# graphdeco-inria/editable-gaussian-reflections

Measured on AMD Instinct MI355X. Metric: Mrays/s fwd+bwd @1080p, 1M Gaussians, higher is better.
Workload: dtype f32; 1 GPU; BASELINE config C: synthetic dense-init room+spheres cloud, HEADLINE variant = init (literal dense-init opacity 0.1 (config.py:44): Kc ~ 22 per ray, bounces mostly die), N=1000000, 1920x1080, one training iteration: export + update_bvh + forward + backward + grad import, num_bounces=2, jitter on, reference default config; variant=init, gaussians=1000000, width=1920, height=1080, parallelism=image tiles x1 + 1 all-reduce of the launch's [22N] gradients, team_help=product default (on)

## Files before the change

editable-gaussian-reflections_amd/csrc/backward_task.inc:

```
        const uint32_t task = v.bwd_order[tq];
        uint32_t blk = v.task_last_block[(size_t)step * (BATCH ? v.num_tasks * v.batch_frames : v.num_tasks) + task];
        if (blk == 0xFFFFFFFFu) continue;
        uint32_t tb = task, bframe = 0u;
        if constexpr (BATCH) tb = batch_base_task(v, task), bframe = v.batch_frame0 + (task >> v.task_shift) % v.batch_frames;
        (void)bframe;
        const TaskGeom tg = task_geom(v, tb, lane);
        const StateRef S = state_of(v, task, lane);
        uint32_t steps_done = tg.inside ? f2u(S.ld(F_STEPS)) : 0u;
        uint32_t nhits = (tg.inside && (uint32_t)step < steps_done && blk != 0xFFFFFFFFu) ? f2u(S.ld(SF(step, S_NHITS))) : 0u;
        const uint32_t max_hits = wave_max_u32(nhits);
        if (max_hits == 0) continue;
#if defined(EGR_TASK_TIMES) && EGR_TASK_TIMES == 8
        if (PRIMARY) bw_rows0 = max_hits;
#endif

        f3 dL_rgb = mk3(0, 0, 0), dL_n = mk3(0, 0, 0), dL_f0 = mk3(0, 0, 0);
        float dL_depth = 0.0f, dL_rough = 0.0f;
        f3 ro = mk3(0, 0, 0), rd = mk3(0, 0, 1);
        f3 rem_rgb = mk3(0, 0, 0), rem_n = mk3(0, 0, 0), rem_f0 = mk3(0, 0, 0);
        float rem_depth = 0.0f, rem_rough = 0.0f, T_minus_Ttot = 0.0f;
        if (nhits > 0) {
            const uint32_t pid = tg.pixel_id;
            const float third = 1.0f / 3.0f;
            if (PRIMARY && BATCH) {
// ... 18 lines not shown
                dL_rgb = mk3(third * sign1(o_rgb.x - td[0]), third * sign1(o_rgb.y - td[1]), third * sign1(o_rgb.z - td[2])) * *v.cfg.loss_weight_diffuse;
                dL_depth = sign1(o_depth - v.fb.target_depth[pid]) * *v.cfg.loss_weight_depth;
                dL_n = mk3(third * sign1(o_n.x - tn[0]), third * sign1(o_n.y - tn[1]), third * sign1(o_n.z - tn[2])) * *v.cfg.loss_weight_normal;
                dL_f0 = mk3(third * sign1(o_f0.x - tf[0]), third * sign1(o_f0.y - tf[1]), third * sign1(o_f0.z - tf[2])) * *v.cfg.loss_weight_f0;
                dL_rough = sign1(o_rough - v.fb.target_roughness[pid]) * *v.cfg.loss_weight_roughness;
                uint32_t seed = tea4(pid, (uint32_t)*v.meta.total_num_calls);
                ro = mk3(v.cam.origin[0], v.cam.origin[1], v.cam.origin[2]);
                rd = primary_direction(v, tg.px, tg.py, *v.cfg.jitter_primary_rays != 0, seed, view_size, v.cam.rotation_w2c);
            } else {
                f3 spec = mk3(0, 0, 0);
                for (int j = 1; j < num_bounces + 1; j++)
                    if ((uint32_t)j < steps_done) spec = spec + S.ld3(SF(j, S_RGB));
                f3 t_spec;
                if constexpr (BATCH) {
                    const float *p = v.batch_targets[1];
                    const size_t P = v.num_pixels, q = (size_t)bframe * 3 * P + pid;
                    t_spec = p ? mk3(p[q], p[q + P], p[q + 2 * P]) : mk3(0, 0, 0);
                } else {
                    const float *ts = v.fb.target_specular + 3 * (size_t)pid;
                    t_spec = mk3(ts[0], ts[1], ts[2]);
                }
                float down = powf(1.0f - S.ld(SF(step - 1, S_ROUGH)), EGR_ROUGHNESS_DOWNWEIGHT_GRAD_POWER);
                dL_rgb = (mk3(third * sign1(spec.x - t_spec.x), third * sign1(spec.y - t_spec.y), third * sign1(spec.z - t_spec.z)) *
                          *v.cfg.loss_weight_specular) * down;
                dL_rgb = dL_rgb * S.ld3(SF(step - 1, S_THR));
                ro = S.ld3(SF(step - 1, S_NEXT_O));
                rd = S.ld3(SF(step - 1, S_NEXT_D));
            }
            rem_rgb = S.ld3(SF(step, S_REM_RGB)), rem_n = S.ld3(SF(step, S_REM_NORMAL)), rem_f0 = S.ld3(SF(step, S_REM_F0));
            rem_depth = S.ld(SF(step, S_REM_DEPTH)), rem_rough = S.ld(SF(step, S_REM_ROUGH));
            T_minus_Ttot = S.ld(SF(step, S_T)) - S.ld(SF(step, S_TTOT));
        }

        auto hit_geometry = [&](uint32_t pos, const float4 &a2, const f3 &ro, const f3 &rd, float dL_dalpha, auto &gx) { hit_geometry_fn(v, exp_power, eps_scale_grad, pos, a2, ro, rd, dL_dalpha, gx); };

        if constexpr (!PRIMARY) {
            table_dirty = true;
            bdl[lane] = dL_rgb.x, bdl[EGR_WAVE + lane] = dL_rgb.y, bdl[2 * EGR_WAVE + lane] = dL_rgb.z;
            bray[lane] = ro.x, bray[EGR_WAVE + lane] = ro.y, bray[2 * EGR_WAVE + lane] = ro.z, bray[3 * EGR_WAVE + lane] = rd.x, bray[4 * EGR_WAVE + lane] = rd.y, bray[5 * EGR_WAVE + lane] = rd.z;
            f3 prev_rgb = mk3(0, 0, 0), w_rgb = mk3(0, 0, 0);
            const uint32_t nblocks = (max_hits + EGR_HIT_BLOCK_ROWS - 1) / EGR_HIT_BLOCK_ROWS;
            EGR_BWD_SYNC();
            for (uint32_t b = nblocks; b-- > 0;) {
                const float4 *rows = v.hit_arena + (size_t)blk * (EGR_HIT_BLOCK_ROWS + 1) * EGR_WAVE;
                for (int chunk = EGR_HIT_BLOCK_ROWS / 4 - 1; chunk >= 0; chunk--) {
                    uint32_t nitems = 0u;
                    float4 rec4[4], a04[4];
#pragma unroll
                    for (int r4 = 0; r4 < 4; r4++) rec4[r4] = rows[(size_t)(1 + 4 * chunk + r4) * EGR_WAVE + lane];
#pragma unroll
                    for (int r4 = 0; r4 < 4; r4++) a04[r4] = v.app[2 * ((b * EGR_HIT_BLOCK_ROWS + (uint32_t)(4 * chunk + r4)) < nhits ? f2u(rec4[r4].x) : 0u)];
#pragma unroll
                    for (int r4 = 3; r4 >= 0; r4--) {
                        const int row = 4 * chunk + r4;
                        const uint32_t it = b * EGR_HIT_BLOCK_ROWS + (uint32_t)row;
                        const bool act = it < nhits;
                        float dL_dalpha = 0.0f, weight = 0.0f;
                        uint32_t pos = 0u;
                        if (act) {
                            const float4 rec = rec4[r4];
                            pos = f2u(rec.x);
                            const float alpha = rec.z, transmittance = rec.w;
                            weight = (float)((double)transmittance / (1.0 - (double)alpha) * (double)alpha);
                            const float4 a0 = a04[r4];
                            const f3 g_rgb = mk3(a0.x, a0.y, a0.z);
                            w_rgb = w_rgb + (g_rgb - prev_rgb) * transmittance;
                            prev_rgb = g_rgb;
// ... 51 lines not shown
            float4 rec_pf = make_float4(0.f, 0.f, 0.f, 0.f);
            for (int row = EGR_HIT_BLOCK_ROWS - 1; row >= 0; row--) {
                const uint32_t it = b * EGR_HIT_BLOCK_ROWS + (uint32_t)row;
                if (it >= max_hits) continue;
                bool direct = false, want = false;
                uint32_t dpos = 0;
                float gx[EGR_GT_COMPS];
                EGR_BT(const unsigned long long bt0 = __builtin_amdgcn_s_memtime(); unsigned long long bt1 = bt0; bt_rows++;)
                float4 rec_cur = rec_pf;
                const bool have_pf = pf_row == row;
                if (row > 0) {
                    if (it <= nhits) rec_pf = rows[(size_t)row * EGR_WAVE + lane];
                    pf_row = row - 1;
                }
                if (!have_pf) {
                    if (it < nhits) rec_cur = rows[(size_t)(1 + row) * EGR_WAVE + lane];
#if defined(__HIP_DEVICE_COMPILE__)
                    asm volatile("" ::"v"(rec_cur.x), "v"(rec_cur.y), "v"(rec_cur.z), "v"(rec_cur.w));
#endif
                }
                if (it < nhits) {
                    const float4 rec = rec_cur;
                    const uint32_t pos = f2u(rec.x);
                    const float distance = rec.y, alpha = rec.z, transmittance = rec.w;
                    const float4 a0 = v.app[2 * pos], a1 = v.app[2 * pos + 1], a2 = v.inst_w[4 * pos + 3];
                    const f3 g_rgb = mk3(a0.x, a0.y, a0.z);
                    const float weight = (float)((double)transmittance / (1.0 - (double)alpha) * (double)alpha);
                    f3 d_rgb = (dL_rgb * weight);
                    f3 d_n = dL_n * weight, d_f0 = dL_f0 * weight;
                    float d_rough = dL_rough * weight;

                    w_rgb = w_rgb + (g_rgb - prev_rgb) * transmittance;
                    prev_rgb = g_rgb;
                    if (PRIMARY) {
                        f3 g_n = mk3(a0.w, a1.x, a1.y), g_f0 = mk3(a1.z, a1.w, a2.x);
                        w_n = w_n + (g_n - prev_n) * transmittance;
                        prev_n = g_n;
                        w_f0 = w_f0 + (g_f0 - prev_f0) * transmittance;
                        prev_f0 = g_f0;
                        w_rough += (a2.y - prev_rough) * transmittance;
                        prev_rough = a2.y;
                        w_depth += (distance - prev_depth) * transmittance;
                        prev_depth = distance;
                    }
                    float dL_dalpha = 0.0f;
                    const float one_m_alpha = 1.0f - alpha, r1ma = egr_rcp_refined(one_m_alpha);
                    const float tmp1 = egr_div_rn(1.0f, one_m_alpha, r1ma);
                    dL_dalpha += dot(w_rgb * tmp1, dL_rgb);
                    dL_dalpha += dot(w_n * tmp1, dL_n);
                    dL_dalpha += dot(w_f0 * tmp1, dL_f0);
                    dL_dalpha += (w_rough * tmp1) * dL_rough;
                    dL_dalpha += (w_depth * tmp1) * dL_depth;
                    const float tmp2 = -egr_div_rn(T_minus_Ttot, one_m_alpha, r1ma);
                    dL_dalpha += tmp2 * dot(rem_rgb, dL_rgb);
                    dL_dalpha += tmp2 * dot(rem_n, dL_n);
                    dL_dalpha += tmp2 * dot(rem_f0, dL_f0);
                    dL_dalpha += tmp2 * (rem_rough * dL_rough);
                    dL_dalpha += tmp2 * (rem_depth * dL_depth);

                    hit_geometry(pos, a2, ro, rd, dL_dalpha, gx);
                    gx[GC_RGB] = d_rgb.x, gx[GC_RGB + 1] = d_rgb.y, gx[GC_RGB + 2] = d_rgb.z, gx[GC_WEIGHT] = weight;
                    gx[GC_NORMAL] = d_n.x, gx[GC_NORMAL + 1] = d_n.y, gx[GC_NORMAL + 2] = d_n.z;
                    gx[GC_F0] = d_f0.x, gx[GC_F0 + 1] = d_f0.y, gx[GC_F0 + 2] = d_f0.z, gx[GC_ROUGH] = d_rough;
                    EGR_BT(bt1 = __builtin_amdgcn_s_memtime();)
                    dpos = pos;
                    if (PRIMARY) want = primary_presum(pos, gx, lane);
                    else direct = true;
                }
                if (PRIMARY) direct = primary_table_add(v, want, dpos, gx, gt_keys, gt_vals, gt_claim, stage, lane, records);
                EGR_BT(const unsigned long long bt2 = __builtin_amdgcn_s_memtime(); bt_math += bt1 - bt0; bt_table += bt2 - bt1;)
                if (__ballot(direct) != 0ull) {
                    float lo[15];
#pragma unroll
                    for (int c = 0; c < 15; c++) lo[c] = gx[c];
                    wide_add_wave(v, direct, dpos, lo, 0u, stage);
                    if (PRIMARY) {
                        float hi[15];
#pragma unroll
                        for (int c = 0; c < 15; c++) hi[c] = (15 + c < EGR_GT_COMPS) ? gx[(15 + c < EGR_GT_COMPS) ? 15 + c : 0] : 0.0f;
                        wide_add_wave(v, direct, dpos, hi, 15u, stage);
                        records += 2u * (uint32_t)__popcll(__ballot(direct));
                    } else {
                        records += (uint32_t)__popcll(__ballot(direct));
                    }
                }
                EGR_BT(bt_wide += __builtin_amdgcn_s_memtime() - bt2;)
            }
            blk = f2u(rows[0].x);
        }
        EGR_BT(const unsigned long long bt3 = __builtin_amdgcn_s_memtime();)
        if (PRIMARY) records += grad_table_flush(v, gt_keys, gt_vals, stage, lane);
#ifdef EGR_TRAVERSAL_STATS
        if (lane == 0) {
            unsigned long long *d = reinterpret_cast<unsigned long long *>(v.control + CW_DBG2 + 16 + (PRIMARY ? 0 : 10));
            atomicAdd(d, bt_math), atomicAdd(d + 1, bt_table), atomicAdd(d + 2, bt_wide), atomicAdd(d + 3, __builtin_amdgcn_s_memtime() - bt3), atomicAdd(d + 4, bt_rows);
        }
#endif
#undef EGR_BT
```

editable-gaussian-reflections_amd/csrc/trace.hip:

```cpp
#include <algorithm>
#include <cstdio>
#include <cstdlib>
#include <type_traits>
#include <utility>
#include <vector>

#define EGR_CONTRACT_AFTER_EPILOGUE
#include "egr_epilogue.hpp"

#ifndef EGR_GPOP
#define EGR_GPOP 5
#endif
#define EGR_WALK_MAX_LEAVES (8 * EGR_GPOP * EGR_WIDTH)
#define EGR_LBUF (64 + 2 * EGR_WALK_MAX_LEAVES)
#ifndef EGR_FPOP
#define EGR_FPOP 2
#endif
#ifndef EGR_PSTK
#define EGR_PSTK 512
#endif

namespace {

EGR_DI uint32_t wave_next_task(uint32_t *heads, uint32_t num_tasks, uint32_t &cur_q, int lane) {
// ... 19 lines not shown
}
EGR_DI uint32_t wave_max_u32(uint32_t x) {
#pragma unroll
    for (int off = 32; off > 0; off >>= 1) x = max(x, (uint32_t)__shfl_xor((int)x, off));
    return x;
}
EGR_DI void add64(uint32_t *ctrl, int word, uint32_t x) {
    if (x) atomicAdd(reinterpret_cast<unsigned long long *>(ctrl + word), (unsigned long long)x);
}

EGR_DI f3 primary_direction(const DeviceView &v, int ix, int iy, bool jitter, uint32_t &seed, const float view_size, const float *w2c) {
    float aspect_ratio = (float)v.width / (float)v.height;
    float fx = (float)ix, fy = (float)iy;
    if (jitter) {
        float jx = rnd(seed) - 0.5f;
        float jy = rnd(seed) - 0.5f;
        fx += jx;
        fy += jy;
    }
    float y = view_size * (1.0f - 2.0f * (fy + 0.5f) / (float)v.height);
    float x = aspect_ratio * view_size * (2.0f * (fx + 0.5f) / (float)v.width - 1.0f);
    const float *w = w2c;
    f3 w0 = mk3(w[0], w[1], w[2]), w1 = mk3(w[3], w[4], w[5]), w2 = mk3(w[6], w[7], w[8]);
    return normalize(w0 * x + w1 * y - w2);
}

#pragma clang fp contract(off)
EGR_DI float egr_dot3(float ax, float ay, float az, float bx, float by, float bz) {
    return __builtin_fmaf(az, bz, __builtin_fmaf(ax, bx, ay * by));
}
EGR_DI float egr_madd(float a, float b, float c) {
    return __builtin_fmaf(a, b, c);
}
EGR_DI f3 egr_div3_rn(const f3 &a, const f3 &b, const f3 &r) { return mk3(egr_div_rn(a.x, b.x, r.x), egr_div_rn(a.y, b.y, r.y), egr_div_rn(a.z, b.z, r.z)); }
EGR_DI float egr_gaussian_sq(float sq, float exp_power) {
    const float two_p = 2.0f * exp_power;
    return expf(egr_div_rn(-pow_exp(sq, exp_power), two_p, egr_rcp_refined(two_p)));
}
EGR_DI f3 object_origin(const float4 &w0, const float4 &w1, const float4 &w2, const f3 &o) {
    f3 lo;
    lo.x = egr_dot3(w0.x, w0.y, w0.z, o.x, o.y, o.z) + w0.w, lo.y = egr_dot3(w1.x, w1.y, w1.z, o.x, o.y, o.z) + w1.w, lo.z = egr_dot3(w2.x, w2.y, w2.z, o.x, o.y, o.z) + w2.w;
    return lo;
}
EGR_DI void candidate_geometry_from(const float4 &w0, const float4 &w1, const float4 &w2, const f3 &lo, const f3 &d, f3 &ld, f3 &dhat, float &t, f3 &u, bool &behind,
                                    bool &outside) {
    ld.x = egr_dot3(w0.x, w0.y, w0.z, d.x, d.y, d.z), ld.y = egr_dot3(w1.x, w1.y, w1.z, d.x, d.y, d.z), ld.z = egr_dot3(w2.x, w2.y, w2.z, d.x, d.y, d.z);
    const float norm = egr_sqrt_rn(egr_dot3(ld.x, ld.y, ld.z, ld.x, ld.y, ld.z));
    const float rr = egr_rcp_refined(norm);
    const float inv = egr_div_rn(1.0f, norm, rr);
    dhat.x = ld.x * inv, dhat.y = ld.y * inv, dhat.z = ld.z * inv;
    const float tl = egr_dot3(-lo.x, -lo.y, -lo.z, dhat.x, dhat.y, dhat.z);
    t = egr_div_rn(tl, norm, rr);
    u.x = egr_madd(tl, dhat.x, lo.x), u.y = egr_madd(tl, dhat.y, lo.y), u.z = egr_madd(tl, dhat.z, lo.z);
    behind = egr_dot3(lo.x, lo.y, lo.z, ld.x, ld.y, ld.z) > 0.0f;
    outside = egr_dot3(u.x, u.y, u.z, u.x, u.y, u.z) > 1.0f;
}
EGR_DI void candidate_geometry(const float4 &w0, const float4 &w1, const float4 &w2, const f3 &o, const f3 &d, f3 &lo, f3 &ld, f3 &dhat, float &t, f3 &u,
                               bool &behind, bool &outside) {
    lo = object_origin(w0, w1, w2, o);
    candidate_geometry_from(w0, w1, w2, lo, d, ld, dhat, t, u, behind, outside);
}
#pragma clang fp contract(fast)
typedef float egr_v8f __attribute__((ext_vector_type(8)));
EGR_DI void load_node_uniform(const float4 *nodes, uint32_t un, float4 &n0, float4 &n1) {
#if defined(__HIP_DEVICE_COMPILE__)
    const __attribute__((address_space(4))) egr_v8f *p = (const __attribute__((address_space(4))) egr_v8f *)nodes;
    const egr_v8f x = p[un];
// ... 416 lines not shown
    float4 *app = v.app + 2 * pos;
    app[0] = make_float4(relu_act(g.rgb[3 * i]), relu_act(g.rgb[3 * i + 1]), relu_act(g.rgb[3 * i + 2]), g.normal[3 * i]);
    app[1] = make_float4(g.normal[3 * i + 1], g.normal[3 * i + 2], clip01_act(g.f0[3 * i]), clip01_act(g.f0[3 * i + 1]));
    v.inst_w[4 * pos + 3] = make_float4(clip01_act(g.f0[3 * i + 2]), clip01_act(g.roughness[i]), o, sigma);
    if (grads) {
        float4 *im = v.inst_m + 4 * pos;
        im[0].w = expf(g.scale[3 * i]), im[1].w = expf(g.scale[3 * i + 1]), im[2].w = expf(g.scale[3 * i + 2]);
        im[3] = reinterpret_cast<const float4 *>(g.rotation)[i];
    }
}

#ifndef EGR_ARENA_CHUNK
#define EGR_ARENA_CHUNK 8
#endif
#ifndef EGR_FWD_WAVES
#define EGR_FWD_WAVES 4
#endif
template <bool GRADS, bool CUBE, int TEAM> __global__ void __launch_bounds__(EGR_WAVE * TEAM) __attribute__((amdgpu_waves_per_eu(EGR_FWD_WAVES, EGR_FWD_WAVES))) k_forward_chain(DeviceView v) {
    constexpr bool BATCH = false;
#include "forward_chain.inc"
}
template <bool CUBE, int TEAM> __global__ void __launch_bounds__(EGR_WAVE * TEAM) __attribute__((amdgpu_waves_per_eu(EGR_FWD_WAVES, EGR_FWD_WAVES))) k_forward_batch(DeviceView v) {
    constexpr bool GRADS = false, BATCH = true;
#include "forward_chain.inc"
}
template <bool CUBE, int TEAM> __global__ void __launch_bounds__(EGR_WAVE * TEAM) __attribute__((amdgpu_waves_per_eu(EGR_FWD_WAVES, EGR_FWD_WAVES))) k_forward_batch_grads(DeviceView v) {
    constexpr bool GRADS = true, BATCH = true;
#include "forward_chain.inc"
}

#ifndef EGR_GT_SLOTS
#define EGR_GT_SLOTS 80
#endif
#define EGR_GT_COMPS 22
#define EGR_GT_STRIDE 23
#define EGR_GT_EMPTY 0xFFFFFFFFu
enum : int { GC_OPA = 0, GC_SCALE = 1, GC_MEAN = 4, GC_ROT = 7, GC_RGB = 11, GC_WEIGHT = 14, GC_NORMAL = 15, GC_F0 = 18, GC_ROUGH = 21 };
#define EGR_ROW_STRIDE 32
#define EGR_BWD_SYNC() wave_sync()

EGR_DI void wide_add_wave(const DeviceView &v, bool ok, uint32_t pos, const float (&r)[15], uint32_t base, float4 *stage) {
    const int lane = threadIdx.x & (EGR_WAVE - 1);
    if (ok) {
        stage[4 * lane + 0] = make_float4(u2f(pos), r[0], r[1], r[2]);
        stage[4 * lane + 1] = make_float4(r[3], r[4], r[5], r[6]);
        stage[4 * lane + 2] = make_float4(r[7], r[8], r[9], r[10]);
        stage[4 * lane + 3] = make_float4(r[11], r[12], r[13], r[14]);
    }
    const unsigned long long okm = __ballot(ok);
    EGR_BWD_SYNC();
    const float *sf = reinterpret_cast<const float *>(stage);
#pragma unroll 4
    for (int pass = 0; pass < 16; pass++) {
        const int src = 4 * pass + (lane >> 4), c = lane & 15;
        if (((okm >> (4 * pass)) & 0xFull) == 0ull) continue;
        const float x = sf[16 * src + c];
        const uint32_t p = f2u(sf[16 * src]);
        if (((okm >> src) & 1ull) && c != 0 && x != 0.0f) atomicAdd(v.grad_rows + (size_t)p * EGR_ROW_STRIDE + base + (uint32_t)(c - 1), x);
    }
    EGR_BWD_SYNC();
}

EGR_DI uint32_t grad_table_flush(const DeviceView &v, uint32_t *gt_keys, float *gt_vals, float4 *stage, int lane) {
    uint32_t sent = 0u;
    EGR_BWD_SYNC();
    for (int s0 = 0; s0 < EGR_GT_SLOTS; s0 += EGR_WAVE) {
        const int s = min(s0 + lane, EGR_GT_SLOTS - 1);
        const bool in_table = s0 + lane < EGR_GT_SLOTS;
        const uint32_t pos = in_table ? gt_keys[s] : EGR_GT_EMPTY;
        const bool valid = pos != EGR_GT_EMPTY;
        if (in_table) gt_keys[s] = EGR_GT_EMPTY;
        float lo[15], hi[15];
#pragma unroll
        for (int c = 0; c < 15; c++) {
            lo[c] = valid ? gt_vals[s * EGR_GT_STRIDE + c] : 0.0f;
            if (valid) gt_vals[s * EGR_GT_STRIDE + c] = 0.0f;
        }
#pragma unroll
        for (int c = 0; c < 15; c++) {
            hi[c] = 0.0f;
            if (15 + c < EGR_GT_COMPS) {
                hi[c] = valid ? gt_vals[s * EGR_GT_STRIDE + 15 + c] : 0.0f;
                if (valid) gt_vals[s * EGR_GT_STRIDE + 15 + c] = 0.0f;
            }
        }
        if (__ballot(valid) == 0ull) continue;
        wide_add_wave(v, valid, pos, lo, 0u, stage);
        wide_add_wave(v, valid, pos, hi, 15u, stage);
        sent += 2u * (uint32_t)__popcll(__ballot(valid));
    }
    EGR_BWD_SYNC();
    return sent;
}

EGR_DI bool primary_presum(const uint32_t pos, float (&gx)[EGR_GT_COMPS], const int lane) {
    bool mine = true;
    {
        const unsigned long long em = __ballot(true);
#define EGR_FETCH_DPP(x, ctrl) __builtin_amdgcn_update_dpp(0, (int)(x), ctrl, 0xF, 0xF, false)
#define EGR_FETCH_SWZ(x, pat) __builtin_amdgcn_ds_swizzle((int)(x), pat)
#define EGR_FETCH_X32(x, unused) __shfl_xor((int)(x), 32)
#define EGR_FETCH_DPP4(x, unused) __builtin_amdgcn_update_dpp(0, __builtin_amdgcn_update_dpp(0, (int)(x), 0x141, 0xF, 0xF, false), 0x1B, 0xF, 0xF, false)
#define EGR_COMBINE(d, FETCH, arg)                                                                            \
    {                                                                                                          \
        const bool pact = ((em >> ((uint32_t)lane ^ (d))) & 1ull) != 0ull;                                     \
        const uint32_t ppos = (uint32_t)FETCH(pos, arg), pmine = (uint32_t)FETCH(mine ? 1 : 0, arg);           \
        const bool same = pact && pmine != 0u && mine && ppos == pos;                                          \
        const bool take = same && ((uint32_t)lane & (d)) == 0u;                                                \
        _Pragma("unroll") for (int c = 0; c < EGR_GT_COMPS; c++) {                                             \
            const float o = __int_as_float(FETCH(__float_as_int(gx[c]), arg));                                 \
            gx[c] += take ? o : 0.0f;                                                                          \
        }                                                                                                      \
        if (same && !take) mine = false;                                                                       \
    }
        EGR_COMBINE(1u, EGR_FETCH_DPP, 0xB1)
        EGR_COMBINE(8u, EGR_FETCH_DPP, 0x128)
#undef EGR_COMBINE
#undef EGR_FETCH_DPP
#undef EGR_FETCH_SWZ
#undef EGR_FETCH_X32
#undef EGR_FETCH_DPP4
// ... 9 lines not shown
        found = false;
#pragma unroll 1
        for (int pr = 0; pr < (want ? 8 : 0); pr++) {
            uint32_t key = *reinterpret_cast<volatile uint32_t *>(&gt_keys[slot]);
            if (key == EGR_GT_EMPTY) key = atomicCAS(&gt_keys[slot], EGR_GT_EMPTY, pos), key = key == EGR_GT_EMPTY ? pos : key;
            if (key == pos) { found = true; break; }
            slot = slot + 1u == (uint32_t)EGR_GT_SLOTS ? 0u : slot + 1u;
        }
    };
    probe();
    if (__ballot(want && !found) != 0ull) {
        records += grad_table_flush(v, gt_keys, gt_vals, stage, lane);
        probe();
    }
    bool pending = found;
    while (__ballot(pending) != 0ull) {
        if (pending) gt_claim[slot] = (uint32_t)lane;
        EGR_BWD_SYNC();
        const bool win = pending && gt_claim[slot] == (uint32_t)lane;
        if (win) {
            float *cell = gt_vals + slot * EGR_GT_STRIDE;
            float cur[EGR_GT_COMPS];
#pragma unroll
            for (int c = 0; c < EGR_GT_COMPS; c++) cur[c] = cell[c];
#pragma unroll
            for (int c = 0; c < EGR_GT_COMPS; c++) cell[c] = cur[c] + gx[c];
            pending = false;
        }
        EGR_BWD_SYNC();
    }
    return want && !found;
}

template <class GX> EGR_DI void hit_geometry_fn(const DeviceView &v, const float exp_power, const float eps_scale_grad, uint32_t pos, const float4 &a2, const f3 &ro, const f3 &rd, float dL_dalpha, GX &gx) {
    const float opacity = a2.z, scaling_factor = a2.w;
    const float4 W0 = v.inst_w[4 * pos], W1 = v.inst_w[4 * pos + 1], W2 = v.inst_w[4 * pos + 2];
    const float4 M0 = v.inst_m[4 * pos], M1 = v.inst_m[4 * pos + 1], M2 = v.inst_m[4 * pos + 2], qu = v.inst_m[4 * pos + 3];
    f3 lo, ld, dhat, u;
    float t_unused;
    bool behind_unused, outside_unused;
    candidate_geometry(W0, W1, W2, ro, rd, lo, ld, dhat, t_unused, u, behind_unused, outside_unused);
    const f3 local_hit = u * scaling_factor;
    const float sq_norm = dot(local_hit, local_hit);
    const float gaussval = egr_gaussian_sq(sq_norm, exp_power);

    float d_opacity = EGR_MAX_ALPHA * dL_dalpha * gaussval;
    d_opacity = d_opacity * opacity * (1.0f - opacity);
    const float dL_dgaussval = EGR_MAX_ALPHA * dL_dalpha * opacity;
    const float dL_dsq_norm = gaussval * pow_exp_m1(sq_norm, exp_power);
    const f3 dL_dx_local = (-local_hit * dL_dsq_norm) * dL_dgaussval;
    const f3 dL_dx_world = mk3(dot(mk3(W0.x, W1.x, W2.x), dL_dx_local), dot(mk3(W0.y, W1.y, W2.y), dL_dx_local),
                               dot(mk3(W0.z, W1.z, W2.z), dL_dx_local)) * scaling_factor;
    const f3 dl2w0 = -dL_dx_world.x * local_hit, dl2w1 = -dL_dx_world.y * local_hit, dl2w2 = -dL_dx_world.z * local_hit;
    const f3 d_mean = -dL_dx_world;
    const f3 scaling = mk3(M0.w, M1.w, M2.w);
    const f3 den = mk3(scaling.x * scaling_factor + eps_scale_grad, scaling.y * scaling_factor + eps_scale_grad,
                       scaling.z * scaling_factor + eps_scale_grad);
    const f3 rden = mk3(egr_rcp_refined(den.x), egr_rcp_refined(den.y), egr_rcp_refined(den.z));
    const f3 rot_0 = egr_div3_rn(mk3(M0.x, M0.y, M0.z), den, rden), rot_1 = egr_div3_rn(mk3(M1.x, M1.y, M1.z), den, rden), rot_2 = egr_div3_rn(mk3(M2.x, M2.y, M2.z), den, rden);
    const f3 d_scale = (dl2w0 * rot_0 + dl2w1 * rot_1 + dl2w2 * rot_2) * scaling;
    const f3 dr0 = dl2w0 * scaling, dr1 = dl2w1 * scaling, dr2 = dl2w2 * scaling;
    const float qn = egr_sqrt_rn(qu.x * qu.x + qu.y * qu.y + qu.z * qu.z + qu.w * qu.w);
    const float rqn = egr_rcp_refined(qn);
    const float r = egr_div_rn(qu.x, qn, rqn), x = egr_div_rn(qu.y, qn, rqn), y = egr_div_rn(qu.z, qn, rqn), z = egr_div_rn(qu.w, qn, rqn);
    const float dL_dr = 2.f * x * (dr2.y - dr1.z) + 2.f * y * (dr0.z - dr2.x) + 2.f * z * (dr1.x - dr0.y);
    const float dL_dx = -4.f * x * (dr1.y + dr2.z) + 2.f * y * (dr0.y + dr1.x) + 2.f * z * (dr0.z + dr2.x) + 2.f * r * (dr2.y - dr1.z);
    const float dL_dy = 2.f * x * (dr0.y + dr1.x) - 4.f * y * (dr0.x + dr2.z) + 2.f * z * (dr1.z + dr2.y) + 2.f * r * (dr0.z - dr2.x);
    const float dL_dz = 2.f * x * (dr0.z + dr2.x) + 2.f * y * (dr1.z + dr2.y) - 4.f * z * (dr0.x + dr1.y) + 2.f * r * (dr1.x - dr0.y);
    const float dd = dL_dr * qu.x + dL_dx * qu.y + dL_dy * qu.z + dL_dz * qu.w;
    const float qn3 = qn * qn * qn;
    const float inv3 = egr_div_rn(1.0f, qn3, egr_rcp_refined(qn3)), inv1 = egr_div_rn(1.0f, qn, rqn);

    const float d_rot0 = dd * -qu.x * inv3 + dL_dr * inv1, d_rot1 = dd * -qu.y * inv3 + dL_dx * inv1;
    const float d_rot2 = dd * -qu.z * inv3 + dL_dy * inv1, d_rot3 = dd * -qu.w * inv3 + dL_dz * inv1;
    gx[GC_OPA] = d_opacity, gx[GC_SCALE] = d_scale.x, gx[GC_SCALE + 1] = d_scale.y, gx[GC_SCALE + 2] = d_scale.z;
    gx[GC_MEAN] = d_mean.x, gx[GC_MEAN + 1] = d_mean.y, gx[GC_MEAN + 2] = d_mean.z;
    gx[GC_ROT] = d_rot0, gx[GC_ROT + 1] = d_rot1, gx[GC_ROT + 2] = d_rot2, gx[GC_ROT + 3] = d_rot3;
}

EGR_DI uint32_t bounce_batch(const DeviceView &v, const float exp_power, const float eps_scale_grad, const uint4 *bitems, const float *bdl, const float *bray, uint32_t i0, uint32_t nitems,
                             float4 *stage, int lane) {
    const bool valid = i0 + (uint32_t)lane < nitems;
    uint32_t dpos = 0;
    float gx[15];
#pragma unroll
    for (int c = 0; c < 15; c++) gx[c] = 0.0f;
    if (valid) {
        const uint4 item = bitems[i0 + (uint32_t)lane];
        const uint32_t ray = item.x, pos = item.z;
        const float weight = u2f(item.w);
        const float4 a2 = v.inst_w[4 * pos + 3];
        const f3 iro = mk3(bray[ray], bray[EGR_WAVE + ray], bray[2 * EGR_WAVE + ray]), ird = mk3(bray[3 * EGR_WAVE + ray], bray[4 * EGR_WAVE + ray], bray[5 * EGR_WAVE + ray]);
        hit_geometry_fn(v, exp_power, eps_scale_grad, pos, a2, iro, ird, u2f(item.y), gx);
        gx[GC_RGB] = bdl[ray] * weight, gx[GC_RGB + 1] = bdl[EGR_WAVE + ray] * weight, gx[GC_RGB + 2] = bdl[2 * EGR_WAVE + ray] * weight;
        gx[GC_WEIGHT] = weight;
        dpos = pos;
    }
    wide_add_wave(v, valid, dpos, gx, 0u, stage);
    return (uint32_t)__popcll(__ballot(valid));
}

#ifndef EGR_BWD_TEAM
#define EGR_BWD_TEAM 4
#endif
template <int TEAM> struct BwdTeamShared {
    uint32_t done;
    uint32_t ticket[TEAM], nitems[TEAM], finished[TEAM];
};

#ifndef EGR_BWD_WAVES
#define EGR_BWD_WAVES 3
#endif
#ifndef EGR_ORDER_BUCKETS
#define EGR_ORDER_BUCKETS 16
#endif
#ifndef EGR_ORDER_SHIFT
#define EGR_ORDER_SHIFT 7
#endif
__global__ void __launch_bounds__(256) k_order_backward(DeviceView v) {
    __shared__ uint32_t cnt[EGR_ORDER_BUCKETS][256 + 1];
    const uint32_t chunk = ((v.num_tasks + 7u) / 8u + 3u) & ~3u, q = blockIdx.x;
    const uint32_t beg = q * chunk, end = min(beg + chunk, v.num_tasks);
    if (beg >= end) return;
    const uint32_t t = threadIdx.x, n = end - beg, per = (n + 255u) / 256u;
    const uint32_t i0 = min(t * per, n), i1 = min(i0 + per, n);
    auto bucket = [](uint32_t cost) { return (uint32_t)EGR_ORDER_BUCKETS - 1u - min(cost >> EGR_ORDER_SHIFT, (uint32_t)EGR_ORDER_BUCKETS - 1u); };
    for (int b = 0; b < EGR_ORDER_BUCKETS; b++) cnt[b][t] = 0u;
    for (uint32_t i = i0; i < i1; i++) cnt[bucket(v.task_cost[beg + i])][t]++;
    __syncthreads();
    if (t < (uint32_t)EGR_ORDER_BUCKETS) {
        uint32_t acc = 0u;
// ... 25 lines not shown
        bool any = false;
        for (int dlt = 1; dlt < TEAM; dlt++) {
            const int w = (wv + dlt) % TEAM;
            const uint32_t peek = uniform_u32(lds_peek(&bteam.ticket[w]));
            if ((peek & 0x3FFu) >= ((peek >> 10) & 0x3FFu)) continue;
            uint32_t tk = 0u;
            if (lane == 0) tk = atomicAdd(&bteam.ticket[w], 1u);
            tk = uniform_u32(tk);
            const uint32_t bi = tk & 0x3FFu, nbatch = (tk >> 10) & 0x3FFu;
            if (bi >= nbatch) continue;
            const uint32_t nitems = uniform_u32(lds_peek(&bteam.nitems[w]));
            const uint4 *bitems = reinterpret_cast<const uint4 *>(gt_vals_all[w]);
            records += bounce_batch(v, exp_power, eps_scale_grad, bitems, gt_vals_all[w] + 16 * EGR_WAVE, gt_vals_all[w] + 19 * EGR_WAVE, bi * (uint32_t)EGR_WAVE, nitems, stage, lane);
            if (lane == 0) atomicAdd(&bteam.finished[w], 1u);
            any = true;
        }
        if (!any) __builtin_amdgcn_s_sleep(2);
    }
    return records;
}

template <int TEAM> __global__ void __launch_bounds__(EGR_WAVE * TEAM) __attribute__((amdgpu_waves_per_eu(EGR_BWD_WAVES, EGR_BWD_WAVES))) k_backward_chain(DeviceView v) {
    constexpr bool BATCH = false;
#include "backward_chain.inc"
}
template <int TEAM> __global__ void __launch_bounds__(EGR_WAVE * TEAM) __attribute__((amdgpu_waves_per_eu(EGR_BWD_WAVES, EGR_BWD_WAVES))) k_backward_batch(DeviceView v) {
    constexpr bool BATCH = true;
#include "backward_chain.inc"
}

template <bool OVERWRITE> __global__ void __launch_bounds__(256) k_grad_gather(DeviceView v) {
    const uint32_t gid = blockIdx.x * 256 + threadIdx.x;
    if (gid >= v.n) return;
    float4 *row = reinterpret_cast<float4 *>(v.grad_rows + (size_t)v.pos_of_gid[gid] * EGR_ROW_STRIDE);
    float x[24];
    uint32_t any = 0;
#pragma unroll
    for (int q = 0; q < 6; q++) {
        const float4 r = row[q];
        x[4 * q] = r.x, x[4 * q + 1] = r.y, x[4 * q + 2] = r.z, x[4 * q + 3] = r.w;
        any |= (f2u(r.x) | f2u(r.y) | f2u(r.z) | f2u(r.w)) << 1;
    }
    if (!OVERWRITE && any == 0) return;
    if (any != 0) {
#pragma unroll
        for (int q = 0; q < 6; q++) row[q] = make_float4(0.f, 0.f, 0.f, 0.f);
    }
    const egr_gaussians &g = v.g;
    auto put = [](float *p, float val) {
        if (OVERWRITE) *p = val;
        else *p += val;
    };
    put(g.dL_dopacity + gid, x[GC_OPA]);
#pragma unroll
    for (int a = 0; a < 3; a++) {
        put(g.dL_dscale + 3 * gid + a, x[GC_SCALE + a]), put(g.dL_dmean + 3 * gid + a, x[GC_MEAN + a]), put(g.dL_drgb + 3 * gid + a, x[GC_RGB + a]);
        put(g.dL_dnormal + 3 * gid + a, x[GC_NORMAL + a]), put(g.dL_df0 + 3 * gid + a, x[GC_F0 + a]);
    }
#pragma unroll
    for (int a = 0; a < 4; a++) put(g.dL_drotation + 4 * gid + a, x[GC_ROT + a]);
    put(g.dL_droughness + gid, x[GC_ROUGH]);
    put(g.total_weight + gid, x[GC_WEIGHT]);
}

__global__ void __launch_bounds__(EGR_WAVE) k_finish(DeviceView v) {
    const int lane = threadIdx.x;
    const bool accumulate = *v.cfg.accumulate_samples != 0;
    const float cnt = accumulate ? (float)(*v.fb.accumulated_sample_count + 1) : 1.0f;
    const size_t P = v.num_pixels;
    for (uint32_t task = blockIdx.x; task < v.num_tasks; task += gridDim.x) {
        const TaskGeom tg = task_geom(v, task, lane);
        if (!tg.inside) continue;
        const StateRef S = state_of(v, task, lane);
        const uint32_t steps = f2u(S.ld(F_STEPS));
        f3 final = mk3(0, 0, 0);
        for (int s = 0; s < EGR_NSTEPS; s++) {
            const bool done = (uint32_t)s < steps;
            f3 rgb = done ? S.ld3(SF(s, S_RGB)) : mk3(0, 0, 0), n = done ? S.ld3(SF(s, S_NORMAL)) : mk3(0, 0, 0);
            f3 f0 = done ? S.ld3(SF(s, S_F0)) : mk3(0, 0, 0);
// ... 605 lines not shown
```

Baseline: 453.1 Mrays/s.

## Defer primary-hit scale/rotation chain rule to per-Gaussian gather via symmetric moments

For primary hits, the backward pass no longer evaluates the per-hit scale and quaternion chain rule. It instead accumulates six symmetric outer-product moments (ql ⊗ local_hit), which shrinks the per-hit record and drops the inst_m loads. k_grad_gather then reconstructs the scale and rotation gradients once per Gaussian in double precision from those moments. This cuts per-hit ALU work and register pressure in the hot loop, at the cost of extra double math and wider row reads in the gather kernel, plus a remapped atomic cell layout.

```diff
diff --git a/editable-gaussian-reflections_amd/csrc/backward_task.inc b/editable-gaussian-reflections_amd/csrc/backward_task.inc
--- a/editable-gaussian-reflections_amd/csrc/backward_task.inc
+++ b/editable-gaussian-reflections_amd/csrc/backward_task.inc
@@ -74,7 +74,7 @@
             T_minus_Ttot = S.ld(SF(step, S_T)) - S.ld(SF(step, S_TTOT));
         }
 
-        auto hit_geometry = [&](uint32_t pos, const float4 &a2, const f3 &ro, const f3 &rd, float dL_dalpha, auto &gx) { hit_geometry_fn(v, exp_power, eps_scale_grad, pos, a2, ro, rd, dL_dalpha, gx); };
+        auto hit_geometry = [&](uint32_t pos, const float4 &a2, const f3 &ro, const f3 &rd, float dL_dalpha, auto &gx) { hit_geometry_fn<true>(v, exp_power, eps_scale_grad, pos, a2, ro, rd, dL_dalpha, gx); };
 
         if constexpr (!PRIMARY) {
             table_dirty = true;
@@ -192,7 +192,7 @@
 
                     w_rgb = w_rgb + (g_rgb - prev_rgb) * transmittance;
                     prev_rgb = g_rgb;
-                    if (PRIMARY) {
+                    {
                         f3 g_n = mk3(a0.w, a1.x, a1.y), g_f0 = mk3(a1.z, a1.w, a2.x);
                         w_n = w_n + (g_n - prev_n) * transmittance;
                         prev_n = g_n;
@@ -219,37 +219,32 @@
                     dL_dalpha += tmp2 * (rem_depth * dL_depth);
 
                     hit_geometry(pos, a2, ro, rd, dL_dalpha, gx);
-                    gx[GC_RGB] = d_rgb.x, gx[GC_RGB + 1] = d_rgb.y, gx[GC_RGB + 2] = d_rgb.z, gx[GC_WEIGHT] = weight;
-                    gx[GC_NORMAL] = d_n.x, gx[GC_NORMAL + 1] = d_n.y, gx[GC_NORMAL + 2] = d_n.z;
-                    gx[GC_F0] = d_f0.x, gx[GC_F0 + 1] = d_f0.y, gx[GC_F0 + 2] = d_f0.z, gx[GC_ROUGH] = d_rough;
+                    gx[PC_RGB] = d_rgb.x, gx[PC_RGB + 1] = d_rgb.y, gx[PC_RGB + 2] = d_rgb.z, gx[PC_WEIGHT] = weight;
+                    gx[PC_NORMAL] = d_n.x, gx[PC_NORMAL + 1] = d_n.y, gx[PC_NORMAL + 2] = d_n.z;
+                    gx[PC_F0] = d_f0.x, gx[PC_F0 + 1] = d_f0.y, gx[PC_F0 + 2] = d_f0.z, gx[PC_ROUGH] = d_rough;
                     EGR_BT(bt1 = __builtin_amdgcn_s_memtime();)
                     dpos = pos;
-                    if (PRIMARY) want = primary_presum(pos, gx, lane);
-                    else direct = true;
-                }
-                if (PRIMARY) direct = primary_table_add(v, want, dpos, gx, gt_keys, gt_vals, gt_claim, stage, lane, records);
+                    want = primary_presum(pos, gx, lane);
+                }
+                direct = primary_table_add(v, want, dpos, gx, gt_keys, gt_vals, gt_claim, stage, lane, records);
                 EGR_BT(const unsigned long long bt2 = __builtin_amdgcn_s_memtime(); bt_math += bt1 - bt0; bt_table += bt2 - bt1;)
                 if (__ballot(direct) != 0ull) {
                     float lo[15];
 #pragma unroll
                     for (int c = 0; c < 15; c++) lo[c] = gx[c];
-                    wide_add_wave(v, direct, dpos, lo, 0u, stage);
-                    if (PRIMARY) {
-                        float hi[15];
-#pragma unroll
-                        for (int c = 0; c < 15; c++) hi[c] = (15 + c < EGR_GT_COMPS) ? gx[(15 + c < EGR_GT_COMPS) ? 15 + c : 0] : 0.0f;
-                        wide_add_wave(v, direct, dpos, hi, 15u, stage);
-                        records += 2u * (uint32_t)__popcll(__ballot(direct));
-                    } else {
-                        records += (uint32_t)__popcll(__ballot(direct));
-                    }
+                    wide_add_wave<REC_PRIMARY_A>(v, direct, dpos, lo, stage);
+                    float hi[15];
+#pragma unroll
+                    for (int c = 0; c < 15; c++) hi[c] = (15 + c < EGR_GT_COMPS) ? gx[(15 + c < EGR_GT_COMPS) ? 15 + c : 0] : 0.0f;
+                    wide_add_wave<REC_PRIMARY_Q>(v, direct, dpos, hi, stage);
+                    records += 2u * (uint32_t)__popcll(__ballot(direct));
                 }
                 EGR_BT(bt_wide += __builtin_amdgcn_s_memtime() - bt2;)
             }
             blk = f2u(rows[0].x);
         }
         EGR_BT(const unsigned long long bt3 = __builtin_amdgcn_s_memtime();)
-        if (PRIMARY) records += grad_table_flush(v, gt_keys, gt_vals, stage, lane);
+        records += grad_table_flush(v, gt_keys, gt_vals, stage, lane);
 #ifdef EGR_TRAVERSAL_STATS
         if (lane == 0) {
             unsigned long long *d = reinterpret_cast<unsigned long long *>(v.control + CW_DBG2 + 16 + (PRIMARY ? 0 : 10));
diff --git a/editable-gaussian-reflections_amd/csrc/trace.hip b/editable-gaussian-reflections_amd/csrc/trace.hip
--- a/editable-gaussian-reflections_amd/csrc/trace.hip
+++ b/editable-gaussian-reflections_amd/csrc/trace.hip
@@ -75,7 +75,6 @@
 EGR_DI float egr_madd(float a, float b, float c) {
     return __builtin_fmaf(a, b, c);
 }
-EGR_DI f3 egr_div3_rn(const f3 &a, const f3 &b, const f3 &r) { return mk3(egr_div_rn(a.x, b.x, r.x), egr_div_rn(a.y, b.y, r.y), egr_div_rn(a.z, b.z, r.z)); }
 EGR_DI float egr_gaussian_sq(float sq, float exp_power) {
     const float two_p = 2.0f * exp_power;
     return expf(egr_div_rn(-pow_exp(sq, exp_power), two_p, egr_rcp_refined(two_p)));
@@ -558,15 +557,25 @@
 #ifndef EGR_GT_SLOTS
 #define EGR_GT_SLOTS 80
 #endif
-#define EGR_GT_COMPS 22
-#define EGR_GT_STRIDE 23
+#define EGR_GT_COMPS 21
+#define EGR_GT_STRIDE 21
 #define EGR_GT_EMPTY 0xFFFFFFFFu
-enum : int { GC_OPA = 0, GC_SCALE = 1, GC_MEAN = 4, GC_ROT = 7, GC_RGB = 11, GC_WEIGHT = 14, GC_NORMAL = 15, GC_F0 = 18, GC_ROUGH = 21 };
+enum : int { GC_OPA = 0, GC_SCALE = 1, GC_MEAN = 4, GC_ROT = 7, GC_RGB = 11, GC_WEIGHT = 14, GC_NORMAL = 15, GC_F0 = 18, GC_ROUGH = 21, GC_Q = 22 };
+enum : int { PC_OPA = 0, PC_MEAN = 1, PC_RGB = 4, PC_WEIGHT = 7, PC_NORMAL = 8, PC_F0 = 11, PC_ROUGH = 14, PC_Q = 15 };
+enum : int { REC_BOUNCE = 0, REC_PRIMARY_A = 1, REC_PRIMARY_Q = 2 };
 #define EGR_ROW_STRIDE 32
 #define EGR_BWD_SYNC() wave_sync()
 
-EGR_DI void wide_add_wave(const DeviceView &v, bool ok, uint32_t pos, const float (&r)[15], uint32_t base, float4 *stage) {
+template <int REC> EGR_DI void wide_add_wave(const DeviceView &v, bool ok, uint32_t pos, const float (&r)[15], float4 *stage) {
     const int lane = threadIdx.x & (EGR_WAVE - 1);
+    uint32_t cell = 0u;
+    if constexpr (REC == REC_PRIMARY_A) {
+        constexpr int cells[15] = {GC_OPA, GC_MEAN, GC_MEAN + 1, GC_MEAN + 2, GC_RGB, GC_RGB + 1, GC_RGB + 2, GC_WEIGHT, GC_NORMAL, GC_NORMAL + 1, GC_NORMAL + 2, GC_F0, GC_F0 + 1, GC_F0 + 2, GC_ROUGH};
+#pragma unroll
+        for (int i = 0; i < 15; i++) cell = (lane & 15) == i + 1 ? (uint32_t)cells[i] : cell;
+    } else {
+        cell = (REC == REC_PRIMARY_Q ? (uint32_t)GC_Q : 0u) + (uint32_t)((lane & 15) - 1);
+    }
     if (ok) {
         stage[4 * lane + 0] = make_float4(u2f(pos), r[0], r[1], r[2]);
         stage[4 * lane + 1] = make_float4(r[3], r[4], r[5], r[6]);
@@ -582,7 +591,7 @@
         if (((okm >> (4 * pass)) & 0xFull) == 0ull) continue;
         const float x = sf[16 * src + c];
         const uint32_t p = f2u(sf[16 * src]);
-        if (((okm >> src) & 1ull) && c != 0 && x != 0.0f) atomicAdd(v.grad_rows + (size_t)p * EGR_ROW_STRIDE + base + (uint32_t)(c - 1), x);
+        if (((okm >> src) & 1ull) && c != 0 && (REC != REC_PRIMARY_Q || c <= 6) && x != 0.0f) atomicAdd(v.grad_rows + (size_t)p * EGR_ROW_STRIDE + cell, x);
     }
     EGR_BWD_SYNC();
 }
@@ -611,8 +620,8 @@
             }
         }
         if (__ballot(valid) == 0ull) continue;
-        wide_add_wave(v, valid, pos, lo, 0u, stage);
-        wide_add_wave(v, valid, pos, hi, 15u, stage);
+        wide_add_wave<REC_PRIMARY_A>(v, valid, pos, lo, stage);
+        wide_add_wave<REC_PRIMARY_Q>(v, valid, pos, hi, stage);
         sent += 2u * (uint32_t)__popcll(__ballot(valid));
     }
     EGR_BWD_SYNC();
@@ -688,10 +697,52 @@
     return want && !found;
 }
 
-template <class GX> EGR_DI void hit_geometry_fn(const DeviceView &v, const float exp_power, const float eps_scale_grad, uint32_t pos, const float4 &a2, const f3 &ro, const f3 &rd, float dL_dalpha, GX &gx) {
+template <class T> EGR_DI T chain_rcp(T b) {
+    if constexpr (sizeof(T) == sizeof(float)) return egr_rcp_refined(b);
+    else return T(1) / b;
+}
+template <class T> EGR_DI T chain_div(T a, T b, T r) {
+    if constexpr (sizeof(T) == sizeof(float)) return egr_div_rn(a, b, r);
+    else return a / b;
+}
+template <class T> EGR_DI T chain_sqrt(T x) {
+    if constexpr (sizeof(T) == sizeof(float)) return egr_sqrt_rn(x);
+    else return sqrt(x);
+}
+template <class T> struct ChainVec { T x, y, z; };
+template <class T> EGR_DI void scale_rot_chain(const float4 &M0, const float4 &M1, const float4 &M2, const float4 &qu, const float sigma, const float eps, const ChainVec<T> &dl2w0,
+                                               const ChainVec<T> &dl2w1, const ChainVec<T> &dl2w2, T (&d_scale)[3], T (&d_rot)[4]) {
+    const T scaling_factor = sigma, eps_scale_grad = eps;
+    const ChainVec<T> scaling = {T(M0.w), T(M1.w), T(M2.w)};
+    const ChainVec<T> den = {scaling.x * scaling_factor + eps_scale_grad, scaling.y * scaling_factor + eps_scale_grad, scaling.z * scaling_factor + eps_scale_grad};
+    const ChainVec<T> rden = {chain_rcp(den.x), chain_rcp(den.y), chain_rcp(den.z)};
+    auto div3 = [&](const float4 &m) { return ChainVec<T>{chain_div(T(m.x), den.x, rden.x), chain_div(T(m.y), den.y, rden.y), chain_div(T(m.z), den.z, rden.z)}; };
+    const ChainVec<T> rot_0 = div3(M0), rot_1 = div3(M1), rot_2 = div3(M2);
+    d_scale[0] = (dl2w0.x * rot_0.x + dl2w1.x * rot_1.x + dl2w2.x * rot_2.x) * scaling.x;
+    d_scale[1] = (dl2w0.y * rot_0.y + dl2w1.y * rot_1.y + dl2w2.y * rot_2.y) * scaling.y;
+    d_scale[2] = (dl2w0.z * rot_0.z + dl2w1.z * rot_1.z + dl2w2.z * rot_2.z) * scaling.z;
+    auto mul3 = [](const ChainVec<T> &a, const ChainVec<T> &b) { return ChainVec<T>{a.x * b.x, a.y * b.y, a.z * b.z}; };
+    const ChainVec<T> dr0 = mul3(dl2w0, scaling), dr1 = mul3(dl2w1, scaling), dr2 = mul3(dl2w2, scaling);
+    const T qr = qu.x, qx = qu.y, qy = qu.z, qz = qu.w;
+    const T qn = chain_sqrt(qr * qr + qx * qx + qy * qy + qz * qz);
+    const T rqn = chain_rcp(qn);
+    const T r = chain_div(qr, qn, rqn), x = chain_div(qx, qn, rqn), y = chain_div(qy, qn, rqn), z = chain_div(qz, qn, rqn);
+    const T dL_dr = T(2) * x * (dr2.y - dr1.z) + T(2) * y * (dr0.z - dr2.x) + T(2) * z * (dr1.x - dr0.y);
+    const T dL_dx = T(-4) * x * (dr1.y + dr2.z) + T(2) * y * (dr0.y + dr1.x) + T(2) * z * (dr0.z + dr2.x) + T(2) * r * (dr2.y - dr1.z);
+    const T dL_dy = T(2) * x * (dr0.y + dr1.x) - T(4) * y * (dr0.x + dr2.z) + T(2) * z * (dr1.z + dr2.y) + T(2) * r * (dr0.z - dr2.x);
+    const T dL_dz = T(2) * x * (dr0.z + dr2.x) + T(2) * y * (dr1.z + dr2.y) - T(4) * z * (dr0.x + dr1.y) + T(2) * r * (dr1.x - dr0.y);
+    const T dd = dL_dr * qr + dL_dx * qx + dL_dy * qy + dL_dz * qz;
+    const T qn3 = qn * qn * qn;
+    const T inv3 = chain_div(T(1), qn3, chain_rcp(qn3)), inv1 = chain_div(T(1), qn, rqn);
+    d_rot[0] = dd * -qr * inv3 + dL_dr * inv1, d_rot[1] = dd * -qx * inv3 + dL_dx * inv1;
+    d_rot[2] = dd * -qy * inv3 + dL_dy * inv1, d_rot[3] = dd * -qz * inv3 + dL_dz * inv1;
+}
+
+template <bool PRIMARY_HIT, class GX> EGR_DI void hit_geometry_fn(const DeviceView &v, const float exp_power, const float eps_scale_grad, uint32_t pos, const float4 &a2, const f3 &ro, const f3 &rd, float dL_dalpha, GX &gx) {
     const float opacity = a2.z, scaling_factor = a2.w;
     const float4 W0 = v.inst_w[4 * pos], W1 = v.inst_w[4 * pos + 1], W2 = v.inst_w[4 * pos + 2];
-    const float4 M0 = v.inst_m[4 * pos], M1 = v.inst_m[4 * pos + 1], M2 = v.inst_m[4 * pos + 2], qu = v.inst_m[4 * pos + 3];
+    float4 M0, M1, M2, qu;
+    if constexpr (!PRIMARY_HIT) M0 = v.inst_m[4 * pos], M1 = v.inst_m[4 * pos + 1], M2 = v.inst_m[4 * pos + 2], qu = v.inst_m[4 * pos + 3];
     f3 lo, ld, dhat, u;
     float t_unused;
     bool behind_unused, outside_unused;
@@ -707,31 +758,20 @@
     const f3 dL_dx_local = (-local_hit * dL_dsq_norm) * dL_dgaussval;
     const f3 dL_dx_world = mk3(dot(mk3(W0.x, W1.x, W2.x), dL_dx_local), dot(mk3(W0.y, W1.y, W2.y), dL_dx_local),
                                dot(mk3(W0.z, W1.z, W2.z), dL_dx_local)) * scaling_factor;
-    const f3 dl2w0 = -dL_dx_world.x * local_hit, dl2w1 = -dL_dx_world.y * local_hit, dl2w2 = -dL_dx_world.z * local_hit;
     const f3 d_mean = -dL_dx_world;
-    const f3 scaling = mk3(M0.w, M1.w, M2.w);
-    const f3 den = mk3(scaling.x * scaling_factor + eps_scale_grad, scaling.y * scaling_factor + eps_scale_grad,
-                       scaling.z * scaling_factor + eps_scale_grad);
-    const f3 rden = mk3(egr_rcp_refined(den.x), egr_rcp_refined(den.y), egr_rcp_refined(den.z));
-    const f3 rot_0 = egr_div3_rn(mk3(M0.x, M0.y, M0.z), den, rden), rot_1 = egr_div3_rn(mk3(M1.x, M1.y, M1.z), den, rden), rot_2 = egr_div3_rn(mk3(M2.x, M2.y, M2.z), den, rden);
-    const f3 d_scale = (dl2w0 * rot_0 + dl2w1 * rot_1 + dl2w2 * rot_2) * scaling;
-    const f3 dr0 = dl2w0 * scaling, dr1 = dl2w1 * scaling, dr2 = dl2w2 * scaling;
-    const float qn = egr_sqrt_rn(qu.x * qu.x + qu.y * qu.y + qu.z * qu.z + qu.w * qu.w);
-    const float rqn = egr_rcp_refined(qn);
-    const float r = egr_div_rn(qu.x, qn, rqn), x = egr_div_rn(qu.y, qn, rqn), y = egr_div_rn(qu.z, qn, rqn), z = egr_div_rn(qu.w, qn, rqn);
-    const float dL_dr = 2.f * x * (dr2.y - dr1.z) + 2.f * y * (dr0.z - dr2.x) + 2.f * z * (dr1.x - dr0.y);
-    const float dL_dx = -4.f * x * (dr1.y + dr2.z) + 2.f * y * (dr0.y + dr1.x) + 2.f * z * (dr0.z + dr2.x) + 2.f * r * (dr2.y - dr1.z);
-    const float dL_dy = 2.f * x * (dr0.y + dr1.x) - 4.f * y * (dr0.x + dr2.z) + 2.f * z * (dr1.z + dr2.y) + 2.f * r * (dr0.z - dr2.x);
-    const float dL_dz = 2.f * x * (dr0.z + dr2.x) + 2.f * y * (dr1.z + dr2.y) - 4.f * z * (dr0.x + dr1.y) + 2.f * r * (dr1.x - dr0.y);
-    const float dd = dL_dr * qu.x + dL_dx * qu.y + dL_dy * qu.z + dL_dz * qu.w;
-    const float qn3 = qn * qn * qn;
-    const float inv3 = egr_div_rn(1.0f, qn3, egr_rcp_refined(qn3)), inv1 = egr_div_rn(1.0f, qn, rqn);
-
-    const float d_rot0 = dd * -qu.x * inv3 + dL_dr * inv1, d_rot1 = dd * -qu.y * inv3 + dL_dx * inv1;
-    const float d_rot2 = dd * -qu.z * inv3 + dL_dy * inv1, d_rot3 = dd * -qu.w * inv3 + dL_dz * inv1;
-    gx[GC_OPA] = d_opacity, gx[GC_SCALE] = d_scale.x, gx[GC_SCALE + 1] = d_scale.y, gx[GC_SCALE + 2] = d_scale.z;
-    gx[GC_MEAN] = d_mean.x, gx[GC_MEAN + 1] = d_mean.y, gx[GC_MEAN + 2] = d_mean.z;
-    gx[GC_ROT] = d_rot0, gx[GC_ROT + 1] = d_rot1, gx[GC_ROT + 2] = d_rot2, gx[GC_ROT + 3] = d_rot3;
+    if constexpr (PRIMARY_HIT) {
+        gx[PC_OPA] = d_opacity, gx[PC_MEAN] = d_mean.x, gx[PC_MEAN + 1] = d_mean.y, gx[PC_MEAN + 2] = d_mean.z;
+        const f3 ql = -dL_dx_local * scaling_factor;
+        gx[PC_Q] = ql.x * local_hit.x, gx[PC_Q + 1] = ql.x * local_hit.y, gx[PC_Q + 2] = ql.x * local_hit.z;
+        gx[PC_Q + 3] = ql.y * local_hit.y, gx[PC_Q + 4] = ql.y * local_hit.z, gx[PC_Q + 5] = ql.z * local_hit.z;
+    } else {
+        const f3 dl2w0 = -dL_dx_world.x * local_hit, dl2w1 = -dL_dx_world.y * local_hit, dl2w2 = -dL_dx_world.z * local_hit;
+        float d_scale[3], d_rot[4];
+        scale_rot_chain<float>(M0, M1, M2, qu, scaling_factor, eps_scale_grad, {dl2w0.x, dl2w0.y, dl2w0.z}, {dl2w1.x, dl2w1.y, dl2w1.z}, {dl2w2.x, dl2w2.y, dl2w2.z}, d_scale, d_rot);
+        gx[GC_OPA] = d_opacity, gx[GC_SCALE] = d_scale[0], gx[GC_SCALE + 1] = d_scale[1], gx[GC_SCALE + 2] = d_scale[2];
+        gx[GC_MEAN] = d_mean.x, gx[GC_MEAN + 1] = d_mean.y, gx[GC_MEAN + 2] = d_mean.z;
+        gx[GC_ROT] = d_rot[0], gx[GC_ROT + 1] = d_rot[1], gx[GC_ROT + 2] = d_rot[2], gx[GC_ROT + 3] = d_rot[3];
+    }
 }
 
 EGR_DI uint32_t bounce_batch(const DeviceView &v, const float exp_power, const float eps_scale_grad, const uint4 *bitems, const float *bdl, const float *bray, uint32_t i0, uint32_t nitems,
@@ -747,12 +787,12 @@
         const float weight = u2f(item.w);
         const float4 a2 = v.inst_w[4 * pos + 3];
         const f3 iro = mk3(bray[ray], bray[EGR_WAVE + ray], bray[2 * EGR_WAVE + ray]), ird = mk3(bray[3 * EGR_WAVE + ray], bray[4 * EGR_WAVE + ray], bray[5 * EGR_WAVE + ray]);
-        hit_geometry_fn(v, exp_power, eps_scale_grad, pos, a2, iro, ird, u2f(item.y), gx);
+        hit_geometry_fn<false>(v, exp_power, eps_scale_grad, pos, a2, iro, ird, u2f(item.y), gx);
         gx[GC_RGB] = bdl[ray] * weight, gx[GC_RGB + 1] = bdl[EGR_WAVE + ray] * weight, gx[GC_RGB + 2] = bdl[2 * EGR_WAVE + ray] * weight;
         gx[GC_WEIGHT] = weight;
         dpos = pos;
     }
-    wide_add_wave(v, valid, dpos, gx, 0u, stage);
+    wide_add_wave<REC_BOUNCE>(v, valid, dpos, gx, stage);
     return (uint32_t)__popcll(__ballot(valid));
 }
 
@@ -844,11 +884,12 @@
 template <bool OVERWRITE> __global__ void __launch_bounds__(256) k_grad_gather(DeviceView v) {
     const uint32_t gid = blockIdx.x * 256 + threadIdx.x;
     if (gid >= v.n) return;
-    float4 *row = reinterpret_cast<float4 *>(v.grad_rows + (size_t)v.pos_of_gid[gid] * EGR_ROW_STRIDE);
-    float x[24];
-    uint32_t any = 0;
-#pragma unroll
-    for (int q = 0; q < 6; q++) {
+    const size_t pos = v.pos_of_gid[gid];
+    float4 *row = reinterpret_cast<float4 *>(v.grad_rows + pos * EGR_ROW_STRIDE);
+    float x[EGR_ROW_STRIDE];
+    uint32_t any = 0, any_l = 0;
+#pragma unroll
+    for (int q = 0; q < EGR_ROW_STRIDE / 4; q++) {
         const float4 r = row[q];
         x[4 * q] = r.x, x[4 * q + 1] = r.y, x[4 * q + 2] = r.z, x[4 * q + 3] = r.w;
         any |= (f2u(r.x) | f2u(r.y) | f2u(r.z) | f2u(r.w)) << 1;
@@ -856,7 +897,22 @@
     if (!OVERWRITE && any == 0) return;
     if (any != 0) {
 #pragma unroll
-        for (int q = 0; q < 6; q++) row[q] = make_float4(0.f, 0.f, 0.f, 0.f);
+        for (int q = 0; q < EGR_ROW_STRIDE / 4; q++) row[q] = make_float4(0.f, 0.f, 0.f, 0.f);
+    }
+#pragma unroll
+    for (int c = 0; c < 6; c++) any_l |= f2u(x[GC_Q + c]) << 1;
+    if (any_l != 0) {
+        const float4 M0 = v.inst_m[4 * pos], M1 = v.inst_m[4 * pos + 1], M2 = v.inst_m[4 * pos + 2], qu = v.inst_m[4 * pos + 3];
+        const float4 W0 = v.inst_w[4 * pos], W1 = v.inst_w[4 * pos + 1], W2 = v.inst_w[4 * pos + 2];
+        const float scaling_factor = v.inst_w[4 * pos + 3].w;
+        const double q00 = x[GC_Q], q01 = x[GC_Q + 1], q02 = x[GC_Q + 2], q11 = x[GC_Q + 3], q12 = x[GC_Q + 4], q22 = x[GC_Q + 5];
+        auto dl2w_of = [&](double w0, double w1, double w2) { return ChainVec<double>{w0 * q00 + w1 * q01 + w2 * q02, w0 * q01 + w1 * q11 + w2 * q12, w0 * q02 + w1 * q12 + w2 * q22}; };
+        double d_scale[3], d_rot[4];
+        scale_rot_chain<double>(M0, M1, M2, qu, scaling_factor, *v.cfg.eps_scale_grad, dl2w_of(W0.x, W1.x, W2.x), dl2w_of(W0.y, W1.y, W2.y), dl2w_of(W0.z, W1.z, W2.z), d_scale, d_rot);
+#pragma unroll
+        for (int a = 0; a < 3; a++) x[GC_SCALE + a] = (float)((double)x[GC_SCALE + a] + d_scale[a]);
+#pragma unroll
+        for (int a = 0; a < 4; a++) x[GC_ROT + a] = (float)((double)x[GC_ROT + a] + d_rot[a]);
     }
     const egr_gaussians &g = v.g;
     auto put = [](float *p, float val) {
```

Result: faster. 461.0 Mrays/s, median of 6 (+1.7%).
